# YaoChengTang/DecNet

Measured on AMD Instinct MI355X. Metric: stereo pairs/sec at 960x540x192disp (hot path: stage-0 dense + SpaMat/SpaVar stages 1-3), higher is better.
Workload: dtype f32 (bf16x3 on the bf16 matrix pipe); 1 GPU; BASELINE config 2: synthetic 960x540 (padded 972x540), max_disp 192->216: batch=8 synthetic pairs per GPU, feature maps of the 4-stage/scale-3 net, random-init CostRegNetNoDown(216); pairs_per_gpu=8, parallelism=dp1 (pairs sharded, all_gather of disparity maps)

## Files before the change

decnet_amd/csrc/common.h:

```cpp
#pragma once
#include <hip/hip_runtime.h>
#include <stdint.h>

#include "../../include/decnet_hip.h"

#define DECNET_WAVE 64
#define DECNET_LDS_BYTES (160 * 1024)
#define DECNET_LDS_BUDGET (64 * 1024)

static inline int decnet_launch_status() {
    hipError_t e = hipGetLastError();
    return e == hipSuccess ? DECNET_OK : (int)e;
}

static inline int ceil_div(int a, int b) { return (a + b - 1) / b; }

#ifdef __HIPCC__
template <typename K, typename... Args>
static inline int decnet_launch(K kernel, dim3 grid, dim3 block, size_t lds_bytes, hipStream_t stream, Args... args) {
    if (lds_bytes > 64 * 1024) {
        hipError_t e = hipFuncSetAttribute((const void *)kernel, hipFuncAttributeMaxDynamicSharedMemorySize, (int)lds_bytes);
        if (e != hipSuccess) return (int)e;
    }
    hipLaunchKernelGGL(kernel, grid, block, lds_bytes, stream, args...);
    return decnet_launch_status();
}


template <int CF>
__device__ __forceinline__ float decnet_cost(float l, float r) {
#pragma clang fp contract(off)
    if (CF == DECNET_COST_COR) return l * r;
    if (CF == DECNET_COST_SSD) {
        const float volume_sum = l + r;
        const float ll = l * l, rr = r * r;
        const float volume_sqr = ll + rr;
        const float half = volume_sum * 0.5f;
        const float hh = half * half;
        return volume_sqr * 0.5f - hh;
    }
    return l + r;
}

__device__ __forceinline__ bool decnet_xcd_rows(int gx, int nrows, int &bx, int &row) {
    const int T = gx * nrows, per = (T + 7) >> 3;
    const int v = (blockIdx.x & 7) * per + (blockIdx.x >> 3);
    if (v >= T) return false;
    row = v / gx;
    bx = v - row * gx;
    return true;
}
#endif
static inline unsigned decnet_xcd_grid(int gx, long nrows) { return (unsigned)(8 * ((gx * nrows + 7) / 8)); }
```

decnet_amd/csrc/conv3d_winograd.hip:

```cpp
#include <stdlib.h>
#include <string.h>

#include <type_traits>

#include "common.h"


typedef float f32x4 __attribute__((ext_vector_type(4)));
typedef float f32x2 __attribute__((ext_vector_type(2)));
typedef int i32x4 __attribute__((ext_vector_type(4)));
typedef int i32x2 __attribute__((ext_vector_type(2)));

namespace {

constexpr int W_BN = 224;
__host__ __device__ constexpr int pad16(int c) { return (c + 15) & ~15; }

template <int T> __device__ __forceinline__ void bt_1d(float (&v)[T]);
template <> __device__ __forceinline__ void bt_1d<4>(float (&v)[4]) {
    const float t0 = v[0] - v[2], t1 = v[1] + v[2], t2 = v[2] - v[1], t3 = v[1] - v[3];
    v[0] = t0; v[1] = t1; v[2] = t2; v[3] = t3;
}
template <> __device__ __forceinline__ void bt_1d<6>(float (&v)[6]) {
    const float a0 = v[0], a1 = v[1], a2 = v[2], a3 = v[3], a4 = v[4], a5 = v[5];
    const float e = a4 - 2.25f * a2, o = 0.75f * a3 - 1.6875f * a1;
    const float f = a4 - 0.5625f * a2, q = 1.5f * a3 - 0.84375f * a1;
    v[0] = 1.265625f * a0 - 2.8125f * a2 + a4;
    v[1] = e + o;
    v[2] = e - o;
    v[3] = f + q;
    v[4] = f - q;
    v[5] = 1.265625f * a1 - 2.8125f * a3 + a5;
}
template <int T> __device__ __forceinline__ void g_1d(const float (&g)[3], float (&o)[T]);
template <> __device__ __forceinline__ void g_1d<4>(const float (&g)[3], float (&o)[4]) {
    o[0] = g[0]; o[1] = 0.5f * (g[0] + g[1] + g[2]); o[2] = 0.5f * (g[0] - g[1] + g[2]); o[3] = g[2];
}
template <> __device__ __forceinline__ void g_1d<6>(const float (&g)[3], float (&o)[6]) {
    const float ea = (-128.f / 243.f) * (g[0] + 0.5625f * g[2]), oa = (-96.f / 243.f) * g[1];
    const float eb = (32.f / 243.f) * (g[0] + 2.25f * g[2]), ob = (48.f / 243.f) * g[1];
    o[0] = (64.f / 81.f) * g[0];
    o[1] = ea + oa;
    o[2] = ea - oa;
    o[3] = eb + ob;
    o[4] = eb - ob;
    o[5] = g[2];
}
template <int T> __device__ __forceinline__ void at_1d(const float (&m)[T], float (&o)[T - 2]);
template <> __device__ __forceinline__ void at_1d<4>(const float (&m)[4], float (&o)[2]) {
    o[0] = m[0] + m[1] + m[2];
    o[1] = m[1] - m[2] - m[3];
}
template <> __device__ __forceinline__ void at_1d<6>(const float (&m)[6], float (&o)[4]) {
    const float s12 = m[1] + m[2], d12 = m[1] - m[2], s34 = m[3] + m[4], d34 = m[3] - m[4];
    o[0] = m[0] + s12 + s34;
    o[1] = 0.75f * d12 + 1.5f * d34;
    o[2] = 0.5625f * s12 + 2.25f * s34;
    o[3] = 0.421875f * d12 + 3.375f * d34 + m[5];
}

template <int TD, int TH, int TW>
__global__ void wino_weight_transform(const float *__restrict__ w, float *__restrict__ U, int Co,
                                      int Ci) {
    const int idx = blockIdx.x * blockDim.x + threadIdx.x;
// ... 319 lines not shown
#pragma unroll
    for (int i = 0; i < T; ++i) {
        const int z = z0 - 1 + i;
#pragma unroll
        for (int jj = 0; jj < T; ++jj) {
            const int y = y0 - 1 + jj;
            const bool okzy = (unsigned)z < (unsigned)g.D && (unsigned)y < (unsigned)g.H;
            const float *row = ys + ((okzy ? z * g.H + y : 0) * NCH + ch) * Wp;
            float r[T];
#pragma unroll
            for (int k = 0; k < T; ++k) {
                const int x = x0 - 1 + k;
                const bool ok = okzy && (unsigned)x < (unsigned)g.W;
                const float v = row[ok ? x : 0];
                r[k] = ok ? v : 0.f;
            }
            bt_1d<T>(r);
#pragma unroll
            for (int k = 0; k < KW; ++k) d[i][jj][k] = r[K0 + k];
        }
        __builtin_amdgcn_sched_barrier(0);
#pragma unroll
        for (int k = 0; k < KW; ++k) {
            float v[T];
#pragma unroll
            for (int jj = 0; jj < T; ++jj) v[jj] = d[i][jj][k];
            bt_1d<T>(v);
#pragma unroll
            for (int jj = 0; jj < T; ++jj) d[i][jj][k] = v[jj];
        }
        __builtin_amdgcn_sched_barrier(0);
    }
#pragma unroll
    for (int jj = 0; jj < T; ++jj) {
        int xo = xs;
        asm volatile("" : "+s"(xo));
#pragma unroll
        for (int k = 0; k < KW; ++k) {
            float v[T];
#pragma unroll
            for (int i = 0; i < T; ++i) v[i] = d[i][jj][k];
            bt_1d<T>(v);
#pragma unroll
            for (int i = 0; i < T; ++i)
                __builtin_amdgcn_raw_buffer_store_b32(__float_as_int(v[i]), vr, voff, ((i * T + jj) * T + K0 + k) * xo, 0);
        }
        __builtin_amdgcn_sched_barrier(0);
    }
}

template <int NCH = 4, int NTHR = MID_THREADS>
__device__ __forceinline__ void wino_output_phase(__amdgpu_buffer_rsrc_t mr, float *__restrict__ ys, const Tiling &g, int Wp,
                                                  int cq, int b, int nts, int nt, int xs, const float *__restrict__ scale,
                                                  const float *__restrict__ shift, int C, int relu, bool res_in, int c0 = 0) {
    constexpr int T = 6, O = 4;
    const int items = nts * NCH;
    for (int it = threadIdx.x; it < items; it += NTHR) {
        const int ch = it % NCH, tl = it / NCH;
        const int co = cq * 4 + c0 + ch;
        int bb, z0, y0, x0;
        tile_coords<O, O, O>(tl, g, bb, z0, y0, x0);
        const int moff = ((cq * nt + b * nts + tl) * 4 + c0 + ch) * 4;
        float acc[O][O][O];
#pragma unroll
        for (int i = 0; i < O; ++i)
#pragma unroll
            for (int jj = 0; jj < O; ++jj)
#pragma unroll
                for (int k = 0; k < O; ++k) acc[i][jj][k] = 0.f;
        float p0[T][T], p1[T][T];
        auto load_plane = [&](float (&p)[T][T], int i) {
            int xo = xs;
            asm volatile("" : "+s"(xo));
            const int so = i * (T * T) * xo;
#pragma unroll
            for (int jj = 0; jj < T; ++jj)
#pragma unroll
                for (int k = 0; k < T; ++k)
                    p[jj][k] = __int_as_float(__builtin_amdgcn_raw_buffer_load_b32(mr, moff, so + (jj * T + k) * xo, 0));
        };
        auto consume = [&](float (&p)[T][T], int i) {
            float a[T][O], h[O][O];
#pragma unroll
            for (int jj = 0; jj < T; ++jj) at_1d<T>(p[jj], a[jj]);
#pragma unroll
            for (int k = 0; k < O; ++k) {
                float m[T], o[O];
#pragma unroll
                for (int jj = 0; jj < T; ++jj) m[jj] = a[jj][k];
                at_1d<T>(m, o);
#pragma unroll
                for (int jj = 0; jj < O; ++jj) h[jj][k] = o[jj];
            }
            const float c0 = AT6_TAB[i][0], c1 = AT6_TAB[i][1], c2 = AT6_TAB[i][2], c3 = AT6_TAB[i][3];
#pragma unroll
            for (int jj = 0; jj < O; ++jj)
#pragma unroll
                for (int k = 0; k < O; ++k) {
                    acc[0][jj][k] = fmaf(c0, h[jj][k], acc[0][jj][k]);
                    acc[1][jj][k] = fmaf(c1, h[jj][k], acc[1][jj][k]);
                    acc[2][jj][k] = fmaf(c2, h[jj][k], acc[2][jj][k]);
                    acc[3][jj][k] = fmaf(c3, h[jj][k], acc[3][jj][k]);
                }
        };
        load_plane(p0, 0);
#pragma unroll 1
        for (int i = 0; i < T; i += 2) {
            load_plane(p1, i + 1);
            __builtin_amdgcn_sched_barrier(0);
            consume(p0, i);
            __builtin_amdgcn_sched_barrier(0);
            if (i + 2 < T) load_plane(p0, i + 2);
            __builtin_amdgcn_sched_barrier(0);
            consume(p1, i + 1);
            __builtin_amdgcn_sched_barrier(0);
        }
        const float sc = co < C ? scale[co] : 0.f, sh = co < C ? shift[co] : 0.f;
#pragma unroll
        for (int i = 0; i < O; ++i)
#pragma unroll
            for (int jj = 0; jj < O; ++jj) {
                const int z = z0 + i, yy = y0 + jj;
                float *row = ys + ((z * g.H + yy) * NCH + ch) * Wp + x0;
#pragma unroll
                for (int k = 0; k < O; ++k) {
                    if (z < g.D && yy < g.H && x0 + k < g.W) {
                        float v = fmaf(acc[i][jj][k], sc, sh);
                        if (relu) v = fmaxf(v, 0.f);
                        if (res_in) v += row[k];
                        row[k] = v;
                    }
                }
            }
    }
}

__global__ __launch_bounds__(MID_THREADS) void wino_mid_transform(
    const float *M, float *V, const float *__restrict__ scale,
    const float *__restrict__ shift, const float *__restrict__ res_in, float *__restrict__ res_out, Tiling g,
    int C, int nt, int relu) {
    extern __shared__ float ys[];
    constexpr int O = 4;
    const int Wp = g.W | 1, vol = g.D * g.H * 4 * Wp;
    const int nq = (C + 3) >> 2, Q = pad16(C) >> 2;
    const int b = blockIdx.x / nq, cq = blockIdx.x - b * nq;
    const int nts = g.Td * g.Th * g.Tw, items = nts * 4;
    const int xs = Q * nt * 16;
    const __amdgpu_buffer_rsrc_t mr = __builtin_amdgcn_make_buffer_rsrc((void *)M, 0, 216 * xs, 0x00020000);
    const __amdgpu_buffer_rsrc_t vr = __builtin_amdgcn_make_buffer_rsrc((void *)V, 0, 216 * xs, 0x00020000);
    const size_t blk = ((size_t)b * nq + cq) * vol;
    if (res_in) {
        for (int i = threadIdx.x * 4; i < vol; i += MID_THREADS * 4) {
            if (i + 4 <= vol) *reinterpret_cast<f32x4 *>(ys + i) = *reinterpret_cast<const f32x4 *>(res_in + blk + i);
            else for (int e = i; e < vol; ++e) ys[e] = res_in[blk + e];
        }
        __syncthreads();
    }
    wino_output_phase(mr, ys, g, Wp, cq, b, nts, nt, xs, scale, shift, C, relu, res_in != nullptr);
    __syncthreads();
    if (res_out) {
        for (int i = threadIdx.x * 4; i < vol; i += MID_THREADS * 4) {
            if (i + 4 <= vol) *reinterpret_cast<f32x4 *>(res_out + blk + i) = *reinterpret_cast<const f32x4 *>(ys + i);
            else for (int e = i; e < vol; ++e) res_out[blk + e] = ys[e];
        }
    }
    const int itp = (items + 63) & ~63;
    for (int it = threadIdx.x; it < 2 * itp; it += MID_THREADS) {
        const int half = it >= itp, id = it - half * itp;
        if (id >= items) continue;
        const int ch = id & 3, tl = id >> 2;
        int bb, z0, y0, x0;
        tile_coords<O, O, O>(tl, g, bb, z0, y0, x0);
        const int voff = ((cq * nt + b * nts + tl) * 4 + ch) * 4;
        if (half == 0) mid_input_half<0>(ys, vr, voff, xs, g, Wp, ch, z0, y0, x0);
        else mid_input_half<1>(ys, vr, voff, xs, g, Wp, ch, z0, y0, x0);
    }
}

__host__ __device__ inline int head_rw_pitch(int W, int D) { return ((W + D - 1 + 23) & ~31) + 8; }

template <int CF>
__global__ __launch_bounds__(MID_THREADS) void wino_head_transform(
    const float *__restrict__ left, const float *__restrict__ right, float *__restrict__ V, Tiling g, int C, int nt) {
#pragma clang fp contract(off)
    extern __shared__ float ys[];
    constexpr int O = 4;
    const int D = g.D, H = g.H, W = g.W, Wp = W | 1, vol = D * H * 4 * Wp, plane = H * W;
    const int nq = (C + 3) >> 2, Q = pad16(C) >> 2;
    const int b = blockIdx.x / nq, cq = blockIdx.x - b * nq;
    const int nts = g.Td * g.Th * g.Tw, items = nts * 4;
    const int xs = Q * nt * 16;
    const __amdgpu_buffer_rsrc_t vr = __builtin_amdgcn_make_buffer_rsrc((void *)V, 0, 216 * xs, 0x00020000);
    float *Ls = ys + vol, *Rs = Ls + 4 * plane;
    float *tx = Rs + 4 * plane;
    float *ty = tx + 3 * (W + D);
    const int nch = C - cq * 4 < 4 ? C - cq * 4 : 4;
    const size_t src = ((size_t)b * C + cq * 4) * plane;
    for (int i0 = threadIdx.x; i0 < 4 * plane; i0 += 8 * MID_THREADS) {
        float lv[8], rv[8];
#pragma unroll
        for (int u = 0; u < 8; ++u) {
            const int i = i0 + u * MID_THREADS;
            const bool ok = i < nch * plane;
            lv[u] = ok ? left[src + i] : 0.f;
            rv[u] = ok ? right[src + i] : 0.f;
        }
#pragma unroll
        for (int u = 0; u < 8; ++u) {
            const int i = i0 + u * MID_THREADS;
            if (i < 4 * plane) { Ls[i] = lv[u]; Rs[i] = rv[u]; }
        }
    }
    for (int i = threadIdx.x; i < W + D; i += MID_THREADS) {
        const int xd = i - (D - 1);
        const float cx = (float)xd / ((float)(W - 1.0) / 2.0f) - 1.0f;
        const float ix = ((cx + 1.0f) * (float)W - 1.0f) / 2.0f;
        const float fx = floorf(ix);
        tx[3 * i] = fx; tx[3 * i + 2] = ix - fx; tx[3 * i + 1] = 1.0f - (ix - fx);
    }
    for (int y = threadIdx.x; y < H; y += MID_THREADS) {
        const float cy = (float)y / ((float)(H - 1.0) / 2.0f) - 1.0f;
        const float iy = ((cy + 1.0f) * (float)H - 1.0f) / 2.0f;
        const float fy = floorf(iy);
        ty[3 * y] = fy; ty[3 * y + 2] = iy - fy; ty[3 * y + 1] = 1.0f - (iy - fy);
    }
    __syncthreads();
    const int S = W + D - 1, SP = head_rw_pitch(W, D);
    float *RW = ty + 3 * H;
// ... 406 lines not shown
    const long nchunks = (T + cap - 1) / cap;
    return (int)((T + nchunks - 1) / nchunks);
}

template <int OD, int OH, int OW>
int conv_variant(const float *x, const float *u, const float *scale, const float *shift,
                 const float *residual, float *y, float *workspace, int B, int D, int H, int W, int Ci,
                 int Co, int relu, hipStream_t s) {
    constexpr int TD = OD + 2, TH = OH + 2, TW = OW + 2, NP = TD * TH * TW;
    constexpr int KS = 1;
    Tiling g{D, H, W, ceil_div(D, OD), ceil_div(H, OH), ceil_div(W, OW)};
    const double Td = (double)B * g.Td * g.Th * g.Tw;
    if (Td >= 2147483648.0) return DECNET_ERR_BAD_SHAPE;
    const int T = (int)Td, cmax = Ci > Co ? Ci : Co;
    const int ct = chunk_tiles(T, cmax, NP);
    if ((double)ct * pad16(cmax) * 4 * NP >= 2147483647.0) return DECNET_ERR_UNSUPPORTED;
    float *V = workspace, *M = workspace + (size_t)NP * ct * pad16(Ci);
    for (int t_lo = 0; t_lo < T; t_lo += ct) {
        const int nt = T - t_lo < ct ? T - t_lo : ct;
        const int x_bytes = (int)((size_t)B * D * H * W * Ci * 4);
        const int ith = Ci >= 256 ? 256 : (Ci + 63) / 64 * 64;
        hipLaunchKernelGGL((wino_input_transform<TD, TH, TW, KS>),
                           dim3((unsigned)(8 * ((nt + 7) / 8)), (unsigned)(KS * ceil_div(Ci, ith))), dim3(ith), 0, s,
                           x, V, g, Ci, t_lo, nt, x_bytes);
        int rc = decnet_launch_status();
        if (rc) return rc;
        if ((rc = gemm_dispatch(V, u, M, nt, Ci, Co, NP, s))) return rc;
        const size_t n = (size_t)nt * pad16(Co);
        hipLaunchKernelGGL((wino_output_transform<TD, TH, TW, KS>), dim3((unsigned)((n + 255) / 256), KS),
                           dim3(256), 0, s, M, scale, shift, residual, y, g, Co, relu, t_lo, nt,
                           (int)((size_t)B * D * H * W * Co * 4));
        if ((rc = decnet_launch_status())) return rc;
    }
    return DECNET_OK;
}

size_t stack_lds_bytes(int D, int H, int W) { return (size_t)D * H * 4 * (W | 1) * 4; }
size_t stack_residual_floats(int B, int D, int H, int W, int C) { return (size_t)B * ((C + 3) / 4) * D * H * 4 * (W | 1); }

bool stack_ok(int B, int D, int H, int W, int C, int variant) {
    static const int off = [] { const char *e = getenv("DECNET_WINO_STACK"); return e && !strcmp(e, "0") ? 1 : 0; }();
    if (off || variant != 2 || !gemm_bf16x3() || C != 216) return false;
    if (stack_lds_bytes(D, H, W) > 160 * 1024) return false;
    const double T = (double)B * ceil_div(D, 4) * ceil_div(H, 4) * ceil_div(W, 4);
    if (T >= 2147483648.0 || chunk_tiles((int)T, C, 216) < (int)T) return false;
    return (double)T * pad16(C) * 4 * 216 < 2147483647.0 && (double)B * D * H * W * C * 4 < 2147483647.0;
}

static int stack_inplace() {
    static const int k = [] { const char *e = getenv("DECNET_WINO_INPLACE"); return e && !strcmp(e, "0") ? 0 : 1; }();
    return k;
}

size_t head_lds_bytes(int D, int H, int W) {
    return stack_lds_bytes(D, H, W) + ((size_t)8 * H * W + 3 * (W + D) + 3 * H + 4 * H * head_rw_pitch(W, D)) * 4;
}

int conv_stack(const float *x, const float *left, const float *right, const float *const *u,
               const float *const *scale, const float *const *shift,
               int n_layers, int res_src, int res_dst, float *y, float *workspace, float *R, int B, int D, int H,
               int W, int C, hipStream_t s, int cost_func = DECNET_COST_COR) {
    constexpr int NP = 216;
    Tiling g{D, H, W, ceil_div(D, 4), ceil_div(H, 4), ceil_div(W, 4)};
    const int nt = B * g.Td * g.Th * g.Tw;
    float *V = workspace, *M = workspace + (size_t)NP * nt * pad16(C);
    const int bytes = (int)((size_t)B * D * H * W * C * 4);
    const size_t lds = stack_lds_bytes(D, H, W);
    if (hipFuncSetAttribute((const void *)wino_mid_transform, hipFuncAttributeMaxDynamicSharedMemorySize, (int)lds) != hipSuccess) {
        (void)hipGetLastError();
        return DECNET_ERR_UNSUPPORTED;
    }
    if (x) {
        const int ith = C >= 256 ? 256 : (C + 63) / 64 * 64;
        hipLaunchKernelGGL((wino_input_transform<6, 6, 6, 1>), dim3((unsigned)(8 * ((nt + 7) / 8)), (unsigned)ceil_div(C, ith)),
                           dim3(ith), 0, s, x, V, g, C, 0, nt, bytes);
    } else {
        const size_t hl = head_lds_bytes(D, H, W);
        const void *fn = cost_func == DECNET_COST_COR   ? (const void *)wino_head_transform<DECNET_COST_COR>
                         : cost_func == DECNET_COST_SSD ? (const void *)wino_head_transform<DECNET_COST_SSD>
                                                        : (const void *)wino_head_transform<DECNET_COST_SUM>;
        if (hipFuncSetAttribute(fn, hipFuncAttributeMaxDynamicSharedMemorySize, (int)hl) != hipSuccess) {
            (void)hipGetLastError();
            return DECNET_ERR_UNSUPPORTED;
        }
        const dim3 grid((unsigned)(B * ((C + 3) / 4)));
        if (cost_func == DECNET_COST_COR)
            hipLaunchKernelGGL(wino_head_transform<DECNET_COST_COR>, grid, dim3(MID_THREADS), hl, s, left, right, V, g, C, nt);
        else if (cost_func == DECNET_COST_SSD)
            hipLaunchKernelGGL(wino_head_transform<DECNET_COST_SSD>, grid, dim3(MID_THREADS), hl, s, left, right, V, g, C, nt);
        else
            hipLaunchKernelGGL(wino_head_transform<DECNET_COST_SUM>, grid, dim3(MID_THREADS), hl, s, left, right, V, g, C, nt);
    }
    int rc = decnet_launch_status();
    if (rc) return rc;
    for (int i = 0; i < n_layers; ++i) {
        const bool last = i == n_layers - 1;
        const int v_quad = i > 0 || !x, m_quad = !last;
        float *Mi = stack_inplace() && v_quad && m_quad ? V : M;
        if ((rc = gemm_dispatch(V, u[i], Mi, nt, C, C, NP, s, v_quad, m_quad))) return rc;
        if (last) {
            const size_t n = (size_t)nt * pad16(C);
            hipLaunchKernelGGL((wino_output_transform<6, 6, 6, 1>), dim3((unsigned)((n + 255) / 256), 1), dim3(256), 0, s,
                               M, scale[i], shift[i], (const float *)nullptr, y, g, C, 1, 0, nt, bytes);
        } else {
            hipLaunchKernelGGL(wino_mid_transform, dim3((unsigned)(B * ((C + 3) / 4))), dim3(MID_THREADS), lds, s, Mi, V,
                               scale[i], shift[i], i == res_dst ? R : (const float *)nullptr,
                               i == res_src ? R : (float *)nullptr, g, C, nt, 1);
        }
        if ((rc = decnet_launch_status())) return rc;
    }
    return DECNET_OK;
}

bool stack_misaligned(const float *const *u, int n_layers, const float *workspace) {
    uintptr_t a = (uintptr_t)workspace;
    for (int i = 0; i < n_layers; ++i) a |= (uintptr_t)u[i];
    return (a & 15) != 0;
}

int variant_points(int variant) { return variant == 0 ? 64 : variant == 1 ? 144 : variant == 2 ? 216 : -1; }

}

extern "C" {

size_t decnet_conv3d_wino_weight_floats(int Ci, int variant) {
    const int np = variant_points(variant);
    if (np < 0 || Ci < 1) return 0;
    const size_t f32 = (size_t)np * pad16(Ci) * W_BN;
    const size_t split = gemm_bf16x3() ? (size_t)np * ((pad16(Ci) / 16 + 1) / 2) * 3 * W_BN * 16 : 0;
    return f32 + split;
}

int decnet_conv3d_wino_pack_weight(const float *w, float *u, int Co, int Ci, int variant, void *stream) {
    if (!w || !u) return DECNET_ERR_NULL_POINTER;
    if ((uintptr_t)u & 15) return DECNET_ERR_MISALIGNED;
    if (Co < 1 || Ci < 1 || variant_points(variant) < 0) return DECNET_ERR_BAD_SHAPE;
    if (Co > W_BN) return DECNET_ERR_UNSUPPORTED;
    const int n = Ci * W_BN;
    if (variant == 0)
        hipLaunchKernelGGL((wino_weight_transform<4, 4, 4>), dim3(ceil_div(n, 128)), dim3(128), 0,
                           (hipStream_t)stream, w, u, Co, Ci);
    else if (variant == 1)
        hipLaunchKernelGGL((wino_weight_transform<4, 6, 6>), dim3(ceil_div(n, 128)), dim3(128), 0,
                           (hipStream_t)stream, w, u, Co, Ci);
    else
        hipLaunchKernelGGL((wino_weight_transform<6, 6, 6>), dim3(ceil_div(n, 128)), dim3(128), 0,
                           (hipStream_t)stream, w, u, Co, Ci);
    int rc = decnet_launch_status();
    if (rc || !gemm_bf16x3()) return rc;
    const int np = variant_points(variant), KC = pad16(Ci) / 16;
    const int nthr = np * ((KC + 1) / 2) * W_BN * 4;
// ... 45 lines not shown
    const int np = variant_points(variant);
    if (B < 1 || D < 1 || H < 1 || W < 1 || Ci < 1 || Co < 1 || np < 0) return 0;
    const int oh = variant == 0 ? 2 : 4, od = variant == 2 ? 4 : 2;
    const double T = (double)B * ((D + od - 1) / od) * ((H + oh - 1) / oh) * ((W + oh - 1) / oh);
    if (T >= 2147483648.0) return 0;
    const int nt = chunk_tiles((int)T, Ci > Co ? Ci : Co, np);
    return (size_t)np * nt * ((size_t)pad16(Ci) + pad16(Co));
}

size_t decnet_conv3d_wino_stack_workspace_floats(int B, int D, int H, int W, int C, int variant) {
    if (B < 1 || D < 1 || H < 1 || W < 1 || C < 1 || !stack_ok(B, D, H, W, C, variant)) return 0;
    const size_t w = decnet_conv3d_wino_workspace_floats(B, D, H, W, C, C, variant);
    return w ? ((w + 63) & ~(size_t)63) + stack_residual_floats(B, D, H, W, C) : 0;
}

int decnet_conv3d_wino_stack_bn_act(const float *x, const float *const *u, const float *const *scale,
                                    const float *const *shift, int n_layers, int res_src, int res_dst, float *y,
                                    float *workspace, int B, int D, int H, int W, int C, int variant, void *stream) {
    if (!x || !u || !scale || !shift || !y || !workspace) return DECNET_ERR_NULL_POINTER;
    if (B < 1 || D < 1 || H < 1 || W < 1 || C < 1 || n_layers < 1) return DECNET_ERR_BAD_SHAPE;
    for (int i = 0; i < n_layers; ++i)
        if (!u[i] || !scale[i] || !shift[i]) return DECNET_ERR_NULL_POINTER;
    if (stack_misaligned(u, n_layers, workspace)) return DECNET_ERR_MISALIGNED;
    if ((res_src < 0) != (res_dst < 0)) return DECNET_ERR_BAD_SHAPE;
    if (res_src >= 0 && !(res_src < res_dst && res_dst < n_layers - 1)) return DECNET_ERR_UNSUPPORTED;
    if (n_layers < 2 || !stack_ok(B, D, H, W, C, variant)) return DECNET_ERR_UNSUPPORTED;
    const size_t w = (decnet_conv3d_wino_workspace_floats(B, D, H, W, C, C, variant) + 63) & ~(size_t)63;
    return conv_stack(x, nullptr, nullptr, u, scale, shift, n_layers, res_src, res_dst, y, workspace, workspace + w, B, D, H,
                      W, C, (hipStream_t)stream);
}

int decnet_costvol_wino_stack_bn_act(const float *left, const float *right, const float *const *u,
                                     const float *const *scale, const float *const *shift, int n_layers, int res_src,
                                     int res_dst, float *y, float *workspace, int B, int C, int H, int W, int D,
                                     int variant, void *stream) {
    return decnet_costvol_wino_stack_bn_act_cf(left, right, u, scale, shift, n_layers, res_src, res_dst, y, workspace, B, C, H,
                                               W, D, variant, DECNET_COST_COR, stream);
}

int decnet_costvol_wino_stack_bn_act_cf(const float *left, const float *right, const float *const *u,
                                        const float *const *scale, const float *const *shift, int n_layers, int res_src,
                                        int res_dst, float *y, float *workspace, int B, int C, int H, int W, int D,
                                        int variant, int cost_func, void *stream) {
    if (!left || !right || !u || !scale || !shift || !y || !workspace) return DECNET_ERR_NULL_POINTER;
    if (B < 1 || D < 1 || H < 1 || W < 1 || C < 1 || n_layers < 1) return DECNET_ERR_BAD_SHAPE;
    if (cost_func != DECNET_COST_COR && cost_func != DECNET_COST_SSD && cost_func != DECNET_COST_SUM)
        return DECNET_ERR_BAD_SHAPE;
    if (H < 2 || W < 2) return DECNET_ERR_UNSUPPORTED;
    for (int i = 0; i < n_layers; ++i)
        if (!u[i] || !scale[i] || !shift[i]) return DECNET_ERR_NULL_POINTER;
    if (stack_misaligned(u, n_layers, workspace)) return DECNET_ERR_MISALIGNED;
    if ((res_src < 0) != (res_dst < 0)) return DECNET_ERR_BAD_SHAPE;
    if (res_src >= 0 && !(res_src < res_dst && res_dst < n_layers - 1)) return DECNET_ERR_UNSUPPORTED;
    static const int off = [] { const char *e = getenv("DECNET_WINO_HEAD"); return e && !strcmp(e, "0") ? 1 : 0; }();
    if (off || n_layers < 2 || !stack_ok(B, D, H, W, C, variant) || head_lds_bytes(D, H, W) > 160 * 1024)
        return DECNET_ERR_UNSUPPORTED;
    const size_t w = (decnet_conv3d_wino_workspace_floats(B, D, H, W, C, C, variant) + 63) & ~(size_t)63;
    return conv_stack(nullptr, left, right, u, scale, shift, n_layers, res_src, res_dst, y, workspace, workspace + w, B, D, H,
                      W, C, (hipStream_t)stream, cost_func);
}

int decnet_conv3d_wino_bn_act(const float *x, const float *u, const float *scale, const float *shift,
                              const float *residual, float *y, float *workspace, int B, int D, int H,
                              int W, int Ci, int Co, int relu, int variant, void *stream) {
    if (!x || !u || !scale || !shift || !y || !workspace) return DECNET_ERR_NULL_POINTER;
    if (((uintptr_t)u | (uintptr_t)workspace) & 15) return DECNET_ERR_MISALIGNED;
    if (B < 1 || D < 1 || H < 1 || W < 1 || Ci < 1 || Co < 1 || variant_points(variant) < 0)
        return DECNET_ERR_BAD_SHAPE;
    if (Ci % 4 != 0 || Co > W_BN) return DECNET_ERR_UNSUPPORTED;
    if ((double)B * D * H * W * (Ci > Co ? Ci : Co) * 4 >= 2147483647.0) return DECNET_ERR_UNSUPPORTED;
    hipStream_t s = (hipStream_t)stream;
    if (variant == 0)
        return conv_variant<2, 2, 2>(x, u, scale, shift, residual, y, workspace, B, D, H, W, Ci, Co, relu, s);
    if (variant == 1)
        return conv_variant<2, 4, 4>(x, u, scale, shift, residual, y, workspace, B, D, H, W, Ci, Co, relu, s);
    return conv_variant<4, 4, 4>(x, u, scale, shift, residual, y, workspace, B, D, H, W, Ci, Co, relu, s);
}

}
```

decnet_amd/csrc/stage0.hip:

```cpp
#include <stdlib.h>
#include <string.h>

#include "common.h"

typedef float f32x4 __attribute__((ext_vector_type(4)));


namespace {

constexpr int CONV_BN = 224;
constexpr int B_PITCH = 240;

template <int CF>
__global__ __launch_bounds__(512) void costvol_ndhwc(const float *__restrict__ left,
                                                     const float *__restrict__ right,
                                                     float *__restrict__ cost, int C, int H,
                                                     int W, int D, int dchunk, int cgn) {
#pragma clang fp contract(off)
    extern __shared__ __attribute__((aligned(16))) float smem[];
    const int WP = W | 1;
    const int c_lo = blockIdx.z * cgn, CN = min(cgn, C - c_lo);
    float *Ls = smem;
    float *R0 = Ls + CN * WP;
    float *R1 = R0 + CN * WP;
// ... 466 lines not shown
#pragma unroll
            for (int t = 0; t < 2; ++t)
                *reinterpret_cast<f32x4_t *>(T + (size_t)p * 32 + t * 16 + kq * 4) = acc[t][0] + acc[t][1];
        }
    }
}

__global__ __launch_bounds__(256) void cout1_gather_softargmax(const float *__restrict__ T, float scale,
                                                               float shift, float *__restrict__ reg,
                                                               float *__restrict__ pred, int B, int D,
                                                               int H, int W, int PB) {
    extern __shared__ float costs[];
    const int npix = B * H * W;
    const int pl = threadIdx.x / D, d = threadIdx.x - pl * D;
    const int pix = blockIdx.x * PB + pl;
    if (pl < PB && pix < npix) {
        const int xx = pix % W, t = pix / W;
        const int yy = t % H, b = t / H;
        float tv[27];
        const size_t centre = ((((size_t)b * D + d) * H + yy) * W + xx) * 32;
#pragma unroll
        for (int tap = 0; tap < 27; ++tap) {
            const int zd = d + tap / 9 - 1, zy = yy + (tap / 3) % 3 - 1, zx = xx + tap % 3 - 1;
            const bool ok = (unsigned)zd < (unsigned)D && (unsigned)zy < (unsigned)H && (unsigned)zx < (unsigned)W;
            tv[tap] = T[ok ? ((((size_t)b * D + zd) * H + zy) * W + zx) * 32 + tap : centre + tap];
        }
        __builtin_amdgcn_sched_barrier(0);
        float acc = 0.f;
#pragma unroll
        for (int tap = 0; tap < 27; ++tap) {
            const int zd = d + tap / 9 - 1, zy = yy + (tap / 3) % 3 - 1, zx = xx + tap % 3 - 1;
            const bool ok = (unsigned)zd < (unsigned)D && (unsigned)zy < (unsigned)H && (unsigned)zx < (unsigned)W;
            acc += ok ? tv[tap] : 0.f;
        }
        const float cost = fmaf(acc, scale, shift);
        costs[pl * D + d] = cost;
        if (reg) reg[(((size_t)b * D + d) * H + yy) * W + xx] = cost;
    }
    __syncthreads();
    if ((int)threadIdx.x < PB && (int)(blockIdx.x * PB + threadIdx.x) < npix) {
        float m = -INFINITY, S = 0.f, Tt = 0.f;
        for (int dd = 0; dd < D; ++dd) {
            const float cost = costs[threadIdx.x * D + dd];
            const float mn = fmaxf(m, cost);
            const float r = expf(m - mn), e = expf(cost - mn);
            S = fmaf(S, r, e);
            Tt = fmaf(Tt, r, e * (float)dd);
            m = mn;
        }
        pred[blockIdx.x * PB + threadIdx.x] = Tt / S;
    }
}

}

extern "C" {

int decnet_costvol_forward(const float *left, const float *right, float *cost, int B, int C, int H,
                           int W, int D, void *stream) {
    return decnet_costvol_forward_cf(left, right, cost, B, C, H, W, D, DECNET_COST_COR, stream);
}

int decnet_costvol_forward_cf(const float *left, const float *right, float *cost, int B, int C, int H,
                              int W, int D, int cost_func, void *stream) {
    if (!left || !right || !cost) return DECNET_ERR_NULL_POINTER;
    if (B < 1 || C < 1 || H < 2 || W < 2 || D < 1 || cost_func < DECNET_COST_COR || cost_func > DECNET_COST_SUM)
        return DECNET_ERR_BAD_SHAPE;
    const int CO = cost_func == DECNET_COST_CAT ? 2 * C : C;
    if ((double)B * D * H * W * CO >= 1099511627776.0 || (double)D * W * CO >= 2147483648.0 ||
        (double)B * H >= 2147483648.0)
        return DECNET_ERR_BAD_SHAPE;
    const int groups = ceil_div(C, 128), cgn = ceil_div(C, groups);
    size_t lds = (size_t)3 * cgn * (W | 1) * 4;
    if (lds > DECNET_LDS_BYTES - 1024) return DECNET_ERR_UNSUPPORTED;
    const void *fn = cost_func == DECNET_COST_COR   ? (const void *)costvol_ndhwc<DECNET_COST_COR>
                     : cost_func == DECNET_COST_SSD ? (const void *)costvol_ndhwc<DECNET_COST_SSD>
                     : cost_func == DECNET_COST_CAT ? (const void *)costvol_ndhwc<DECNET_COST_CAT>
                                                    : (const void *)costvol_ndhwc<DECNET_COST_SUM>;
    if (lds > 64 * 1024) {
        hipError_t e = hipFuncSetAttribute(fn, hipFuncAttributeMaxDynamicSharedMemorySize, (int)lds);
        if (e != hipSuccess) return (int)e;
    }
    int dchunk = 1;
    while (dchunk < D && (long)B * H * ceil_div(C, cgn) * ceil_div(D, 2 * dchunk) >= 512) dchunk *= 2;
    const dim3 grid((unsigned)(B * H), (unsigned)ceil_div(D, dchunk), (unsigned)ceil_div(C, cgn));
#define GO(CF)                                                                                                    \
    hipLaunchKernelGGL(costvol_ndhwc<CF>, grid, dim3(512), lds, (hipStream_t)stream, left, right, cost, C, H, W, D, \
                       dchunk, cgn)
    if (cost_func == DECNET_COST_COR) GO(DECNET_COST_COR);
    else if (cost_func == DECNET_COST_SSD) GO(DECNET_COST_SSD);
    else if (cost_func == DECNET_COST_CAT) GO(DECNET_COST_CAT);
    else GO(DECNET_COST_SUM);
#undef GO
    return decnet_launch_status();
}

static int pointwise_launch(const float *x, const float *w, float *y, const float *x2, const float *w2, float *y2, int B,
                            int Ci, int Co, int P, int ldw, int channels_last, void *stream) {
    if (!x || !w || !y) return DECNET_ERR_NULL_POINTER;
    if (B < 1 || Ci < 1 || Co < 1 || P < 1 || ldw < Ci) return DECNET_ERR_BAD_SHAPE;
    if (B > 65535 || (double)P * (Ci > Co ? Ci : Co) >= 2147483648.0 * 2) return DECNET_ERR_BAD_SHAPE;
    const size_t lds = ((size_t)Ci * PW_TP + (size_t)PW_CK * PW_WP) * 4;
    if (lds > DECNET_LDS_BYTES - 1024) return DECNET_ERR_UNSUPPORTED;
    const void *fn = channels_last ? (const void *)pointwise_conv<true> : (const void *)pointwise_conv<false>;
    if (lds > 64 * 1024) {
        hipError_t e = hipFuncSetAttribute(fn, hipFuncAttributeMaxDynamicSharedMemorySize, (int)lds);
// ... 55 lines not shown
        return launch_conv<4, 24>(x, wp, scale, shift, residual, y, D, H, W, Ci, Co, relu, M, s);
    }
    return launch_conv<2, 24>(x, wp, scale, shift, residual, y, D, H, W, Ci, Co, relu, M, s);
}

int decnet_conv3d_cout1_softargmax(const float *x, const float *w, float scale, float shift,
                                   float *reg, float *pred, int B, int D, int H, int W, int Ci,
                                   void *stream) {
    if (!x || !w || !pred) return DECNET_ERR_NULL_POINTER;
    if (B < 1 || D < 1 || H < 1 || W < 1 || Ci < 1) return DECNET_ERR_BAD_SHAPE;
    if (Ci % 4 != 0) return DECNET_ERR_UNSUPPORTED;
    size_t lds = (size_t)27 * Ci * 4;
    if (lds > DECNET_LDS_BUDGET) return DECNET_ERR_UNSUPPORTED;
    double npix = (double)B * H * W;
    if (npix * D >= 2147483648.0) return DECNET_ERR_BAD_SHAPE;
    int blocks = (int)((npix + 3) / 4);
    if (blocks > 256 * 8) blocks = 256 * 8;
    hipLaunchKernelGGL(conv3d_cout1_softargmax, dim3(blocks), dim3(256), lds, (hipStream_t)stream,
                       x, w, scale, shift, reg, pred, B, D, H, W, Ci);
    return decnet_launch_status();
}

size_t decnet_conv3d_cout1_workspace_floats(int B, int D, int H, int W) {
    if (B < 1 || D < 1 || H < 1 || W < 1) return 0;
    return (size_t)B * D * H * W * 32;
}

int decnet_conv3d_cout1_softargmax_ws(const float *x, const float *w, float scale, float shift,
                                      float *reg, float *pred, float *workspace, int B, int D, int H,
                                      int W, int Ci, void *stream) {
    if (!x || !w || !pred || !workspace) return DECNET_ERR_NULL_POINTER;
    if ((uintptr_t)workspace & 15) return DECNET_ERR_MISALIGNED;
    if (B < 1 || D < 1 || H < 1 || W < 1 || Ci < 1) return DECNET_ERR_BAD_SHAPE;
    const double Md = (double)B * D * H * W;
    if (Ci % 4 != 0 || Ci > 256 || D > 256 || Md * Ci * 4 >= 2147483647.0) return DECNET_ERR_UNSUPPORTED;
    const int M = (int)Md, x_bytes = (int)(Md * Ci * 4);
    hipStream_t s = (hipStream_t)stream;
    int blocks = ceil_div(ceil_div(M, 16), 4);
    if (blocks > 512) blocks = 512;
    if (Ci <= 224 && Ci > 128)
        hipLaunchKernelGGL((cout1_tap_gemm<14>), dim3(blocks), dim3(256), 0, s, x, w, workspace, M, Ci, x_bytes);
    else if (Ci <= 128)
        hipLaunchKernelGGL((cout1_tap_gemm<8>), dim3(blocks), dim3(256), 0, s, x, w, workspace, M, Ci, x_bytes);
    else
        hipLaunchKernelGGL((cout1_tap_gemm<16>), dim3(blocks), dim3(256), 0, s, x, w, workspace, M, Ci, x_bytes);
    int rc = decnet_launch_status();
    if (rc) return rc;
    const int PB = 256 / D, npix = B * H * W;
    hipLaunchKernelGGL(cout1_gather_softargmax, dim3(ceil_div(npix, PB)), dim3(256), (size_t)PB * D * 4, s,
                       workspace, scale, shift, reg, pred, B, D, H, W, PB);
    return decnet_launch_status();
}

int decnet_disparity_regression(const float *cost, const float *samples, float *pred, int B, int S,
                                int H, int W, void *stream) {
    if (!cost || !samples || !pred) return DECNET_ERR_NULL_POINTER;
    if (B < 1 || S < 1 || H < 1 || W < 1) return DECNET_ERR_BAD_SHAPE;
    if ((double)B * S * H * W >= 2147483648.0) return DECNET_ERR_BAD_SHAPE;
    int n = B * H * W;
    hipLaunchKernelGGL(disparity_regression_kernel, dim3(ceil_div(n, 256)), dim3(256), 0,
                       (hipStream_t)stream, cost, samples, pred, B, S, H * W);
    return decnet_launch_status();
}

static int transpose(const float *src, float *dst, int B, int R, int Cn, void *stream) {
    if (!src || !dst) return DECNET_ERR_NULL_POINTER;
    if (B < 1 || R < 1 || Cn < 1 || B > 65535) return DECNET_ERR_BAD_SHAPE;
    if (ceil_div(R, 32) > 65535) return DECNET_ERR_UNSUPPORTED;
    hipLaunchKernelGGL(transpose_inner, dim3(ceil_div(Cn, 32), ceil_div(R, 32), B), dim3(32, 8), 0,
                       (hipStream_t)stream, src, dst, R, Cn);
    return decnet_launch_status();
}

int decnet_ncdhw_to_ndhwc(const float *src, float *dst, int B, int C, int D, int H, int W,
                          void *stream) {
    if (C < 1 || D < 1 || H < 1 || W < 1 || (double)D * H * W >= 2147483648.0)
        return DECNET_ERR_BAD_SHAPE;
    return transpose(src, dst, B, C, D * H * W, stream);
}

int decnet_ndhwc_to_ncdhw(const float *src, float *dst, int B, int C, int D, int H, int W,
                          void *stream) {
    if (C < 1 || D < 1 || H < 1 || W < 1 || (double)D * H * W >= 2147483648.0)
        return DECNET_ERR_BAD_SHAPE;
    return transpose(src, dst, B, D * H * W, C, stream);
}

}
```

decnet_amd/csrc/stage0_entry.hip:

```cpp
#include <stdlib.h>

#include "common.h"

namespace {
inline int auto_variant(int D) { return 216 * ((D + 3) / 4) <= 0.92 * 144 * ((D + 1) / 2) ? 2 : 1; }
inline size_t align64(size_t n) { return (n + 63) & ~(size_t)63; }
constexpr size_t WS_SLACK = 4;
}

extern "C" int decnet_conv3d_pointwise_pair(const float *x, const float *w, float *y, const float *x2, const float *w2,
                                            float *y2, int B, int Ci, int Co, int P, int ldw, void *stream);

extern "C" {

size_t decnet_stage0_cf_workspace_floats(int B, int C, int H, int W, int D, int variant, int cost_func) {
    if (cost_func != DECNET_COST_COR && cost_func != DECNET_COST_SSD && cost_func != DECNET_COST_CAT) return 0;
    const size_t n = decnet_stage0_workspace_floats(B, C, H, W, D, variant);
    return n && cost_func == DECNET_COST_CAT ? n + 2 * align64((size_t)B * C * H * W) : n;
}

size_t decnet_stage0_workspace_floats(int B, int C, int H, int W, int D, int variant) {
    if (B < 1 || C < 1 || H < 1 || W < 1 || D < 1 || variant < -1 || variant > 3) return 0;
    if (variant < 0) variant = auto_variant(D);
    const size_t act = align64((size_t)B * D * H * W * C);
    size_t wino = 0;
    if (variant <= 2) {
        wino = decnet_conv3d_wino_workspace_floats(B, D, H, W, C, C, variant);
        if (!wino) return 0;
        const size_t stack = decnet_conv3d_wino_stack_workspace_floats(B, D, H, W, C, variant);
        if (stack > wino) wino = stack;
    }
    const size_t last = decnet_conv3d_cout1_workspace_floats(B, D, H, W);
    return 4 * act + align64(wino) + (last > act ? align64(last) : 0) + WS_SLACK;
}

int decnet_stage0_forward(const float *left, const float *right, const decnet_stage0_params *p,
                          float *workspace, float *reg, float *pred, int B, int C, int H, int W, int D,
                          int variant, void *stream) {
    return decnet_stage0_forward_cf(left, right, p, nullptr, workspace, reg, pred, B, C, H, W, D, variant, DECNET_COST_COR,
                                    stream);
}

int decnet_stage0_forward_cf(const float *left, const float *right, const decnet_stage0_params *p, const float *w_pre,
                             float *workspace, float *reg, float *pred, int B, int C, int H, int W, int D,
                             int variant, int cost_func, void *stream) {
    if (!left || !right || !p || !workspace || !pred || !p->w_last) return DECNET_ERR_NULL_POINTER;
    if (cost_func != DECNET_COST_COR && cost_func != DECNET_COST_SSD && cost_func != DECNET_COST_CAT)
        return DECNET_ERR_BAD_SHAPE;
    if (cost_func == DECNET_COST_CAT && !w_pre) return DECNET_ERR_NULL_POINTER;
    for (int i = 0; i < 7; ++i)
        if (!p->w[i] || !p->scale[i] || !p->shift[i]) return DECNET_ERR_NULL_POINTER;
    uintptr_t lib_fmt = 0;
    for (int i = 0; i < 7; ++i) lib_fmt |= (uintptr_t)p->w[i];
    if (lib_fmt & 15) return DECNET_ERR_MISALIGNED;
    if (B < 1 || C < 1 || H < 1 || W < 1 || D < 1 || variant < -1 || variant > 3) return DECNET_ERR_BAD_SHAPE;
    if (C % 4) return DECNET_ERR_UNSUPPORTED;
    if (variant < 0) variant = auto_variant(D);
    if (!decnet_stage0_cf_workspace_floats(B, C, H, W, D, variant, cost_func)) return DECNET_ERR_UNSUPPORTED;
    const size_t act = align64((size_t)B * D * H * W * C);
    float *cv = reinterpret_cast<float *>(((uintptr_t)workspace + 15) & ~(uintptr_t)15);
    float *a = cv + act, *b = a + act, *c = b + act, *ws = c + act;
    const size_t stack = variant <= 2 ? decnet_conv3d_wino_stack_workspace_floats(B, D, H, W, C, variant) : 0;
    size_t wino = variant <= 2 ? decnet_conv3d_wino_workspace_floats(B, D, H, W, C, C, variant) : 0;
    wino = align64(stack > wino ? stack : wino);
    const size_t last = decnet_conv3d_cout1_workspace_floats(B, D, H, W);
    float *t_last = last > act ? ws + wino : a;

    int rc;
    int cf = cost_func;
    if (cost_func == DECNET_COST_CAT) {
        if (H < 1 || W < 1 || (double)H * W >= 2147483648.0) return DECNET_ERR_BAD_SHAPE;
        const size_t fm = align64((size_t)B * C * H * W);
        float *pl = ws + wino + (last > act ? align64(last) : 0), *pr = pl + fm;
        if ((rc = decnet_conv3d_pointwise_pair(left, w_pre, pl, right, w_pre + C, pr, B, C, C, H * W, 2 * C, stream))) return rc;
        left = pl;
        right = pr;
        cf = DECNET_COST_SUM;
    }
    rc = DECNET_ERR_UNSUPPORTED;
    if (stack)
        rc = decnet_costvol_wino_stack_bn_act_cf(left, right, p->w, p->scale, p->shift, 7, 1, 4, c, ws, B, C, H, W, D,
                                                 variant, cf, stream);
    if (rc == DECNET_OK) {
        if (C <= 256 && D <= 256)
            return decnet_conv3d_cout1_softargmax_ws(c, p->w_last, p->scale_last, p->shift_last, reg, pred, t_last, B,
                                                     D, H, W, C, stream);
        return decnet_conv3d_cout1_softargmax(c, p->w_last, p->scale_last, p->shift_last, reg, pred, B, D, H, W, C,
                                              stream);
    }
    if (rc != DECNET_ERR_UNSUPPORTED) return rc;
    if ((rc = decnet_costvol_forward_cf(left, right, cv, B, C, H, W, D, cf, stream))) return rc;
    auto conv = [&](int i, const float *src, float *dst, const float *res) {
        if (variant <= 2)
            return decnet_conv3d_wino_bn_act(src, p->w[i], p->scale[i], p->shift[i], res, dst, ws, B, D, H, W, C, C,
                                             1, variant, stream);
        return decnet_conv3d_bn_act(src, p->w[i], p->scale[i], p->shift[i], res, dst, B, D, H, W, C, C, 1, stream);
    };
    rc = DECNET_ERR_UNSUPPORTED;
    if (stack)
        rc = decnet_conv3d_wino_stack_bn_act(cv, p->w, p->scale, p->shift, 7, 1, 4, c, ws, B, D, H, W, C, variant, stream);
    if (rc == DECNET_OK) {
        if (C <= 256 && D <= 256)
            return decnet_conv3d_cout1_softargmax_ws(c, p->w_last, p->scale_last, p->shift_last, reg, pred, t_last, B,
                                                     D, H, W, C, stream);
        return decnet_conv3d_cout1_softargmax(c, p->w_last, p->scale_last, p->shift_last, reg, pred, B, D, H, W, C,
                                              stream);
    }
    if (rc != DECNET_ERR_UNSUPPORTED) return rc;
    if ((rc = conv(0, cv, a, nullptr))) return rc;
    if ((rc = conv(1, a, c, nullptr))) return rc;
    if ((rc = conv(2, c, a, nullptr))) return rc;
    if ((rc = conv(3, a, b, nullptr))) return rc;
    if ((rc = conv(4, b, a, c))) return rc;
    if ((rc = conv(5, a, b, nullptr))) return rc;
    if ((rc = conv(6, b, c, nullptr))) return rc;
    if (C <= 256 && D <= 256)
        return decnet_conv3d_cout1_softargmax_ws(c, p->w_last, p->scale_last, p->shift_last, reg, pred, t_last, B,
                                                 D, H, W, C, stream);
    return decnet_conv3d_cout1_softargmax(c, p->w_last, p->scale_last, p->shift_last, reg, pred, B, D, H, W, C,
                                          stream);
}

}
```

Baseline: 5083 pairs/s.

## Fuse stage-0 last Winograd layer output with Cout=1 conv into tail kernel

Adds a tail path to the Winograd conv stack. The last layer's output transform (BN+ReLU) stays in LDS, and each block applies its 4-channel slice of the final Cout=1 3x3x3 conv there, writing per-quad partial sums. A new reduce kernel sums the partials over channel quads, applies the last scale/shift and computes soft-argmax. This is meant to avoid writing the full C-channel last activation to global memory and reading it back for the separate cout1 conv. In exchange it writes nq partial volumes and needs a full-volume LDS tile, which may hurt occupancy. It is on by default and can be turned off with an environment variable.

```diff
diff --git a/decnet_amd/csrc/common.h b/decnet_amd/csrc/common.h
--- a/decnet_amd/csrc/common.h
+++ b/decnet_amd/csrc/common.h
@@ -14,6 +14,12 @@
 }
 
 static inline int ceil_div(int a, int b) { return (a + b - 1) / b; }
+
+struct decnet_stack_tail {
+    const float *w_last;
+    float scale_last, shift_last;
+    float *reg, *pred, *partial;
+};
 
 #ifdef __HIPCC__
 template <typename K, typename... Args>
diff --git a/decnet_amd/csrc/conv3d_winograd.hip b/decnet_amd/csrc/conv3d_winograd.hip
--- a/decnet_amd/csrc/conv3d_winograd.hip
+++ b/decnet_amd/csrc/conv3d_winograd.hip
@@ -10,6 +10,9 @@
 typedef float f32x2 __attribute__((ext_vector_type(2)));
 typedef int i32x4 __attribute__((ext_vector_type(4)));
 typedef int i32x2 __attribute__((ext_vector_type(2)));
+
+extern "C" int decnet_cout1_reduce_softargmax(const float *P, float scale, float shift, float *reg, float *pred, int B,
+                                              int D, int H, int W, int nq, void *stream);
 
 namespace {
 
@@ -435,9 +438,10 @@
 template <int NCH = 4, int NTHR = MID_THREADS>
 __device__ __forceinline__ void wino_output_phase(__amdgpu_buffer_rsrc_t mr, float *__restrict__ ys, const Tiling &g, int Wp,
                                                   int cq, int b, int nts, int nt, int xs, const float *__restrict__ scale,
-                                                  const float *__restrict__ shift, int C, int relu, bool res_in, int c0 = 0) {
+                                                  const float *__restrict__ shift, int C, int relu, bool res_in, int c0 = 0,
+                                                  int hs = 0) {
     constexpr int T = 6, O = 4;
-    const int items = nts * NCH;
+    const int items = nts * NCH, Hs = hs ? hs : g.H;
     for (int it = threadIdx.x; it < items; it += NTHR) {
         const int ch = it % NCH, tl = it / NCH;
         const int co = cq * 4 + c0 + ch;
@@ -504,7 +508,7 @@
 #pragma unroll
             for (int jj = 0; jj < O; ++jj) {
                 const int z = z0 + i, yy = y0 + jj;
-                float *row = ys + ((z * g.H + yy) * NCH + ch) * Wp + x0;
+                float *row = ys + ((z * Hs + yy) * NCH + ch) * Wp + x0;
 #pragma unroll
                 for (int k = 0; k < O; ++k) {
                     if (z < g.D && yy < g.H && x0 + k < g.W) {
@@ -557,6 +561,69 @@
         const int voff = ((cq * nt + b * nts + tl) * 4 + ch) * 4;
         if (half == 0) mid_input_half<0>(ys, vr, voff, xs, g, Wp, ch, z0, y0, x0);
         else mid_input_half<1>(ys, vr, voff, xs, g, Wp, ch, z0, y0, x0);
+    }
+}
+
+constexpr int TAIL_R = 4;
+__host__ __device__ inline int tail_w_pitch(int W) { return (W + 2) | 1; }
+size_t tail_lds_bytes(int D, int H, int W) { return (size_t)(D + 2) * (H + 2) * 4 * tail_w_pitch(W) * 4; }
+
+__global__ __launch_bounds__(MID_THREADS) void wino_tail_transform(
+    const float *__restrict__ M, const float *__restrict__ scale, const float *__restrict__ shift,
+    const float *__restrict__ w_last, float *__restrict__ P, Tiling g, int C, int nt) {
+    extern __shared__ float ys[];
+    constexpr int R = TAIL_R;
+    const int Wh = tail_w_pitch(g.W), Hh = g.H + 2, vol = (g.D + 2) * Hh * 4 * Wh;
+    const int nq = (C + 3) >> 2, Q = pad16(C) >> 2;
+    const int b = blockIdx.x / nq, cq = blockIdx.x - b * nq;
+    const int nts = g.Td * g.Th * g.Tw;
+    const int xs = Q * nt * 16;
+    const __amdgpu_buffer_rsrc_t mr = __builtin_amdgcn_make_buffer_rsrc((void *)M, 0, 216 * xs, 0x00020000);
+    for (int i = threadIdx.x * 4; i < vol; i += MID_THREADS * 4)
+        *reinterpret_cast<f32x4 *>(ys + i) = f32x4{0.f, 0.f, 0.f, 0.f};
+    __syncthreads();
+    wino_output_phase(mr, ys + (Hh + 1) * 4 * Wh + 1, g, Wh, cq, b, nts, nt, xs, scale, shift, C, 1, false, 0, Hh);
+    __syncthreads();
+    const int nyr = (g.H + R - 1) / R, items = g.D * nyr * g.W;
+    float *__restrict__ pp = P + (size_t)blockIdx.x * g.D * g.H * g.W;
+    const float *__restrict__ wq = w_last + (size_t)cq * 108;
+    for (int it = threadIdx.x; it < items; it += MID_THREADS) {
+        const int x = it % g.W, t = it / g.W;
+        const int z = t / nyr, y0 = (t - z * nyr) * R;
+        int row[R + 2];
+#pragma unroll
+        for (int j = 0; j < R + 2; ++j) row[j] = ((z * Hh + min(y0 + j, Hh - 1)) * 4) * Wh + x;
+        float acc[R];
+#pragma unroll
+        for (int r = 0; r < R; ++r) acc[r] = 0.f;
+#pragma unroll 1
+        for (int ch = 0; ch < 4; ++ch) {
+            float wv[27], v[3][R + 2][3];
+#pragma unroll
+            for (int i = 0; i < 27; ++i) wv[i] = wq[ch * 27 + i];
+#pragma unroll
+            for (int kd = 0; kd < 3; ++kd) {
+                const float *__restrict__ slab = ys + (kd * Hh * 4 + ch) * Wh;
+#pragma unroll
+                for (int j = 0; j < R + 2; ++j)
+#pragma unroll
+                    for (int k = 0; k < 3; ++k) v[kd][j][k] = slab[row[j] + k];
+            }
+#pragma unroll
+            for (int kd = 0; kd < 3; ++kd)
+#pragma unroll
+                for (int j = 0; j < R + 2; ++j)
+#pragma unroll
+                    for (int r = 0; r < R; ++r)
+                        if (j - r >= 0 && j - r < 3) {
+#pragma unroll
+                            for (int k = 0; k < 3; ++k)
+                                acc[r] = fmaf(wv[kd * 9 + (j - r) * 3 + k], v[kd][j][k], acc[r]);
+                        }
+        }
+#pragma unroll
+        for (int r = 0; r < R; ++r)
+            if (y0 + r < g.H) pp[(z * g.H + y0 + r) * g.W + x] = acc[r];
     }
 }
 
@@ -1069,6 +1136,16 @@
     return k;
 }
 
+static int stack_tail_on() {
+    static const int k = [] { const char *e = getenv("DECNET_STAGE0_TAIL"); return e && !strcmp(e, "0") ? 0 : 1; }();
+    return k;
+}
+
+static int head_off() {
+    static const int off = [] { const char *e = getenv("DECNET_WINO_HEAD"); return e && !strcmp(e, "0") ? 1 : 0; }();
+    return off;
+}
+
 size_t head_lds_bytes(int D, int H, int W) {
     return stack_lds_bytes(D, H, W) + ((size_t)8 * H * W + 3 * (W + D) + 3 * H + 4 * H * head_rw_pitch(W, D)) * 4;
 }
@@ -1076,7 +1153,7 @@
 int conv_stack(const float *x, const float *left, const float *right, const float *const *u,
                const float *const *scale, const float *const *shift,
                int n_layers, int res_src, int res_dst, float *y, float *workspace, float *R, int B, int D, int H,
-               int W, int C, hipStream_t s, int cost_func = DECNET_COST_COR) {
+               int W, int C, hipStream_t s, int cost_func = DECNET_COST_COR, const decnet_stack_tail *tail = nullptr) {
     constexpr int NP = 216;
     Tiling g{D, H, W, ceil_div(D, 4), ceil_div(H, 4), ceil_div(W, 4)};
     const int nt = B * g.Td * g.Th * g.Tw;
@@ -1084,6 +1161,11 @@
     const int bytes = (int)((size_t)B * D * H * W * C * 4);
     const size_t lds = stack_lds_bytes(D, H, W);
     if (hipFuncSetAttribute((const void *)wino_mid_transform, hipFuncAttributeMaxDynamicSharedMemorySize, (int)lds) != hipSuccess) {
+        (void)hipGetLastError();
+        return DECNET_ERR_UNSUPPORTED;
+    }
+    const size_t tl = tail_lds_bytes(D, H, W);
+    if (tail && hipFuncSetAttribute((const void *)wino_tail_transform, hipFuncAttributeMaxDynamicSharedMemorySize, (int)tl) != hipSuccess) {
         (void)hipGetLastError();
         return DECNET_ERR_UNSUPPORTED;
     }
@@ -1112,9 +1194,16 @@
     if (rc) return rc;
     for (int i = 0; i < n_layers; ++i) {
         const bool last = i == n_layers - 1;
-        const int v_quad = i > 0 || !x, m_quad = !last;
+        const int v_quad = i > 0 || !x, m_quad = !last || tail;
         float *Mi = stack_inplace() && v_quad && m_quad ? V : M;
         if ((rc = gemm_dispatch(V, u[i], Mi, nt, C, C, NP, s, v_quad, m_quad))) return rc;
+        if (last && tail) {
+            hipLaunchKernelGGL(wino_tail_transform, dim3((unsigned)(B * ((C + 3) / 4))), dim3(MID_THREADS), tl, s, Mi,
+                               scale[i], shift[i], tail->w_last, tail->partial, g, C, nt);
+            if ((rc = decnet_launch_status())) return rc;
+            return decnet_cout1_reduce_softargmax(tail->partial, tail->scale_last, tail->shift_last, tail->reg, tail->pred,
+                                                  B, D, H, W, (C + 3) / 4, s);
+        }
         if (last) {
             const size_t n = (size_t)nt * pad16(C);
             hipLaunchKernelGGL((wino_output_transform<6, 6, 6, 1>), dim3((unsigned)((n + 255) / 256), 1), dim3(256), 0, s,
@@ -1266,12 +1355,34 @@
     if (stack_misaligned(u, n_layers, workspace)) return DECNET_ERR_MISALIGNED;
     if ((res_src < 0) != (res_dst < 0)) return DECNET_ERR_BAD_SHAPE;
     if (res_src >= 0 && !(res_src < res_dst && res_dst < n_layers - 1)) return DECNET_ERR_UNSUPPORTED;
-    static const int off = [] { const char *e = getenv("DECNET_WINO_HEAD"); return e && !strcmp(e, "0") ? 1 : 0; }();
-    if (off || n_layers < 2 || !stack_ok(B, D, H, W, C, variant) || head_lds_bytes(D, H, W) > 160 * 1024)
+    if (head_off() || n_layers < 2 || !stack_ok(B, D, H, W, C, variant) || head_lds_bytes(D, H, W) > 160 * 1024)
         return DECNET_ERR_UNSUPPORTED;
     const size_t w = (decnet_conv3d_wino_workspace_floats(B, D, H, W, C, C, variant) + 63) & ~(size_t)63;
     return conv_stack(nullptr, left, right, u, scale, shift, n_layers, res_src, res_dst, y, workspace, workspace + w, B, D, H,
                       W, C, (hipStream_t)stream, cost_func);
+}
+
+int decnet_wino_stack_tail(const float *x, const float *left, const float *right, const float *const *u,
+                           const float *const *scale, const float *const *shift, int n_layers, int res_src, int res_dst,
+                           const decnet_stack_tail *tail, float *workspace, int B, int C, int H, int W, int D,
+                           int variant, int cost_func, void *stream) {
+    if ((!x && (!left || !right)) || !u || !scale || !shift || !workspace || !tail || !tail->w_last || !tail->pred ||
+        !tail->partial)
+        return DECNET_ERR_NULL_POINTER;
+    if (B < 1 || D < 1 || H < 1 || W < 1 || C < 1 || n_layers < 1) return DECNET_ERR_BAD_SHAPE;
+    if (cost_func != DECNET_COST_COR && cost_func != DECNET_COST_SSD && cost_func != DECNET_COST_SUM)
+        return DECNET_ERR_BAD_SHAPE;
+    for (int i = 0; i < n_layers; ++i)
+        if (!u[i] || !scale[i] || !shift[i]) return DECNET_ERR_NULL_POINTER;
+    if (stack_misaligned(u, n_layers, workspace)) return DECNET_ERR_MISALIGNED;
+    if ((res_src < 0) != (res_dst < 0)) return DECNET_ERR_BAD_SHAPE;
+    if (res_src >= 0 && !(res_src < res_dst && res_dst < n_layers - 1)) return DECNET_ERR_UNSUPPORTED;
+    if (!stack_tail_on() || D > 256 || n_layers < 2 || !stack_ok(B, D, H, W, C, variant)) return DECNET_ERR_UNSUPPORTED;
+    if (tail_lds_bytes(D, H, W) > 160 * 1024) return DECNET_ERR_UNSUPPORTED;
+    if (!x && (H < 2 || W < 2 || head_off() || head_lds_bytes(D, H, W) > 160 * 1024)) return DECNET_ERR_UNSUPPORTED;
+    const size_t w = (decnet_conv3d_wino_workspace_floats(B, D, H, W, C, C, variant) + 63) & ~(size_t)63;
+    return conv_stack(x, left, right, u, scale, shift, n_layers, res_src, res_dst, nullptr, workspace, workspace + w, B, D, H,
+                      W, C, (hipStream_t)stream, cost_func, tail);
 }
 
 int decnet_conv3d_wino_bn_act(const float *x, const float *u, const float *scale, const float *shift,
diff --git a/decnet_amd/csrc/stage0.hip b/decnet_amd/csrc/stage0.hip
--- a/decnet_amd/csrc/stage0.hip
+++ b/decnet_amd/csrc/stage0.hip
@@ -542,6 +542,47 @@
     }
 }
 
+constexpr int REDUCE_BATCH = 54;
+
+__global__ __launch_bounds__(256) void cout1_reduce_softargmax(const float *__restrict__ P, float scale, float shift,
+                                                               float *__restrict__ reg, float *__restrict__ pred,
+                                                               int B, int D, int H, int W, int nq, int PB) {
+    extern __shared__ float costs[];
+    const int HW = H * W, npix = B * HW;
+    const int d = threadIdx.x / PB, pl = threadIdx.x - d * PB;
+    const int pix = blockIdx.x * PB + pl;
+    if (d < D && pix < npix) {
+        const int b = pix / HW, yx = pix - b * HW;
+        const size_t ps = (size_t)D * HW;
+        const float *p = P + ((size_t)b * nq * D + d) * HW + yx;
+        float acc = 0.f;
+        for (int c0 = 0; c0 < nq; c0 += REDUCE_BATCH) {
+            float tv[REDUCE_BATCH];
+#pragma unroll
+            for (int j = 0; j < REDUCE_BATCH; ++j) tv[j] = p[(c0 + j < nq ? c0 + j : nq - 1) * ps];
+            __builtin_amdgcn_sched_barrier(0);
+#pragma unroll
+            for (int j = 0; j < REDUCE_BATCH; ++j) acc += c0 + j < nq ? tv[j] : 0.f;
+        }
+        const float cost = fmaf(acc, scale, shift);
+        costs[d * PB + pl] = cost;
+        if (reg) reg[((size_t)b * D + d) * HW + yx] = cost;
+    }
+    __syncthreads();
+    if ((int)threadIdx.x < PB && (int)(blockIdx.x * PB + threadIdx.x) < npix) {
+        float m = -INFINITY, S = 0.f, Tt = 0.f;
+        for (int dd = 0; dd < D; ++dd) {
+            const float cost = costs[dd * PB + threadIdx.x];
+            const float mn = fmaxf(m, cost);
+            const float r = expf(m - mn), e = expf(cost - mn);
+            S = fmaf(S, r, e);
+            Tt = fmaf(Tt, r, e * (float)dd);
+            m = mn;
+        }
+        pred[blockIdx.x * PB + threadIdx.x] = Tt / S;
+    }
+}
+
 }
 
 extern "C" {
@@ -703,6 +744,17 @@
     return decnet_launch_status();
 }
 
+int decnet_cout1_reduce_softargmax(const float *P, float scale, float shift, float *reg, float *pred, int B, int D,
+                                   int H, int W, int nq, void *stream) {
+    if (!P || !pred) return DECNET_ERR_NULL_POINTER;
+    if (B < 1 || D < 1 || H < 1 || W < 1 || nq < 1) return DECNET_ERR_BAD_SHAPE;
+    if (D > 256 || (double)B * D * H * W >= 2147483648.0) return DECNET_ERR_UNSUPPORTED;
+    const int PB = 256 / D, npix = B * H * W;
+    hipLaunchKernelGGL(cout1_reduce_softargmax, dim3(ceil_div(npix, PB)), dim3(256), (size_t)PB * D * 4,
+                       (hipStream_t)stream, P, scale, shift, reg, pred, B, D, H, W, nq, PB);
+    return decnet_launch_status();
+}
+
 int decnet_disparity_regression(const float *cost, const float *samples, float *pred, int B, int S,
                                 int H, int W, void *stream) {
     if (!cost || !samples || !pred) return DECNET_ERR_NULL_POINTER;
diff --git a/decnet_amd/csrc/stage0_entry.hip b/decnet_amd/csrc/stage0_entry.hip
--- a/decnet_amd/csrc/stage0_entry.hip
+++ b/decnet_amd/csrc/stage0_entry.hip
@@ -10,6 +10,10 @@
 
 extern "C" int decnet_conv3d_pointwise_pair(const float *x, const float *w, float *y, const float *x2, const float *w2,
                                             float *y2, int B, int Ci, int Co, int P, int ldw, void *stream);
+extern "C" int decnet_wino_stack_tail(const float *x, const float *left, const float *right, const float *const *u,
+                                      const float *const *scale, const float *const *shift, int n_layers, int res_src,
+                                      int res_dst, const decnet_stack_tail *tail, float *workspace, int B, int C, int H,
+                                      int W, int D, int variant, int cost_func, void *stream);
 
 extern "C" {
 
@@ -77,10 +81,15 @@
         right = pr;
         cf = DECNET_COST_SUM;
     }
+    const decnet_stack_tail tail{p->w_last, p->scale_last, p->shift_last, reg, pred, a};
     rc = DECNET_ERR_UNSUPPORTED;
-    if (stack)
+    if (stack) {
+        rc = decnet_wino_stack_tail(nullptr, left, right, p->w, p->scale, p->shift, 7, 1, 4, &tail, ws, B, C, H, W, D, variant,
+                                    cf, stream);
+        if (rc != DECNET_ERR_UNSUPPORTED) return rc;
         rc = decnet_costvol_wino_stack_bn_act_cf(left, right, p->w, p->scale, p->shift, 7, 1, 4, c, ws, B, C, H, W, D,
                                                  variant, cf, stream);
+    }
     if (rc == DECNET_OK) {
         if (C <= 256 && D <= 256)
             return decnet_conv3d_cout1_softargmax_ws(c, p->w_last, p->scale_last, p->shift_last, reg, pred, t_last, B,
@@ -97,8 +106,12 @@
         return decnet_conv3d_bn_act(src, p->w[i], p->scale[i], p->shift[i], res, dst, B, D, H, W, C, C, 1, stream);
     };
     rc = DECNET_ERR_UNSUPPORTED;
-    if (stack)
+    if (stack) {
+        rc = decnet_wino_stack_tail(cv, nullptr, nullptr, p->w, p->scale, p->shift, 7, 1, 4, &tail, ws, B, C, H, W, D, variant,
+                                    cf, stream);
+        if (rc != DECNET_ERR_UNSUPPORTED) return rc;
         rc = decnet_conv3d_wino_stack_bn_act(cv, p->w, p->scale, p->shift, 7, 1, 4, c, ws, B, D, H, W, C, variant, stream);
+    }
     if (rc == DECNET_OK) {
         if (C <= 256 && D <= 256)
             return decnet_conv3d_cout1_softargmax_ws(c, p->w_last, p->scale_last, p->shift_last, reg, pred, t_last, B,
```

New measurement: 5118 pairs/s (median of 6 runs). No clear change (+0.7%).
